# Tomsk-Smart-Tech/video-stream-segmenetation

Hardware: AMD Instinct MI355X
Metric: frames/sec (640×480, batch=8) at 1/2/4/8 MI355X + mask max-abs-err vs ref (higher is better)
Workload: dtype bf16; 1 GPU; 8 synthetic 640x480 RGB u8 frames per GPU per step (resident in HBM) -> 256x144 f32 masks, 4 steps in flight (one handle, 4 slots, 4 streams); global_batch=8, frame=640x480x3, model_res=256x144, pw_gemm=v_mfma_f32_16x16x32_bf16, f32 activations split hi+lo, graph=True, inflight=4, parallelism=dp1

## Files before the change

include/vss.h:

```cpp
#ifndef VSS_H_
#define VSS_H_

#include <stddef.h>
#include <stdint.h>

#ifdef __cplusplus
extern "C" {
#endif

#define VSS_VERSION 30000

enum {
  VSS_OK = 0,
  VSS_E_INVALID_ARG = -1,
  VSS_E_HIP = -2,
  VSS_E_RCCL = -3,
  VSS_E_BUSY = -4,
  VSS_E_OOM = -5,
  VSS_E_IO = -6,
  VSS_E_UNSUPPORTED = -7
};

enum {
  VSS_DTYPE_F32 = 0,
// ... 124 lines not shown
int vss_set_option(vss_handle* h, int option, int value);
int vss_get_option(vss_handle* h, int option, int* value);

int vss_layer_shape(const vss_handle* h, int layer, int* c, int* hh, int* ww);

int vss_read_layer(vss_handle* h, int layer, int n, float* host_out);

int vss_layer_kernel(const vss_handle* h, int layer, char* buf, int cap);

int vss_layer_tiles(const vss_handle* h, int layer, int* th, int* tw, int cap);

int vss_layer_tile_kernel(const vss_handle* h, int layer, int idx, char* buf, int cap);

int vss_layer_occupancy(const vss_handle* h, int layer, int* wg_per_cu, int* lds_bytes);

int vss_profile_read(vss_handle* h, double* ms_per_layer, int cap, int* count);

int vss_block_lds_bytes(int mode, int stride, int th, int tw, int cin, int cskip, int chid, int cout, int stem_in);

void vss_expand_frag_layout(int cin, int cout, int* out4);
int vss_expand_frag_image(int cin, int chid, int cout, int h0, int cs, const float* w1, const float* b1,
                          const float* wdw, const float* bdw, const float* w2, void* out);

typedef struct vss_post_config {
  double ema;
  double noise_cutoff;
  double high_threshold;
  double gamma;
  double sigma_spatial;
  double sigma_range;
  int use_bilateral;
} vss_post_config;

void vss_post_config_default(vss_post_config* cfg);

typedef struct vss_post_state vss_post_state;
int vss_post_create(vss_handle* h, const vss_post_config* cfg, vss_post_state** out);
void vss_post_destroy(vss_post_state* st);
int vss_post_reset(vss_post_state* st);
int vss_post_set_config(vss_post_state* st, const vss_post_config* cfg);

int vss_postprocess_device(vss_post_state* st, const uint8_t* d_frames, int n, int height, int width,
                           int channels, size_t row_stride, size_t frame_stride, const float* d_masks,
                           float* d_alpha, uint8_t* d_alpha_u8, void* stream);

typedef struct vss_face_frame {
// ... 54 lines not shown
```

video-stream-segmenetation_amd/__init__.py:

```python
from __future__ import annotations

import ctypes
import os
import subprocess
import threading
import weakref

import numpy as np

HERE = os.path.dirname(os.path.abspath(__file__))
LIB_PATH = os.environ.get("VSS_LIBRARY") or os.path.join(HERE, "lib", "libvss.so")
DEFAULT_WEIGHTS = os.path.join(HERE, "model", "vss_weights_seed7.bin")
HEADER = os.path.join(os.path.dirname(HERE), "include", "vss.h")

VSS_OK, VSS_E_INVALID_ARG, VSS_E_HIP, VSS_E_RCCL, VSS_E_BUSY, VSS_E_OOM, VSS_E_IO, VSS_E_UNSUPPORTED = (
    0, -1, -2, -3, -4, -5, -6, -7)
DTYPES = {"f32": 0, "bf16x2": 1}
VSS_OPT_USE_GRAPH, VSS_OPT_PROFILE, VSS_OPT_KEEP_STEM, VSS_OPT_ROW_FETCH = 1, 2, 6, 7
VSS_OPT_GRAPH_BUILDS, VSS_OPT_GRAPH_PATCHES, VSS_OPT_COMM_RANKS, VSS_OPT_GATHER_CALLS = 8, 9, 10, 11
VSS_OPT_GATHER_FORM = 12
VSS_GATHER_ORDERED, VSS_GATHER_CONCURRENT = 0, 1
GATHER_FORMS = {"ordered": VSS_GATHER_ORDERED, "concurrent": VSS_GATHER_CONCURRENT}
VSS_CREATE_NO_AUTOTUNE = 1
VSS_OUT_MODEL, VSS_OUT_FRAME = 0, 1
# ... 929 lines not shown


def shard_plan(n: int, nranks: int, rank: int):
    f, c, m = ctypes.c_int(), ctypes.c_int(), ctypes.c_int()
    _check(lib().vss_shard_plan(n, nranks, rank, ctypes.byref(f), ctypes.byref(c), ctypes.byref(m)))
    return f.value, c.value, m.value


def gather_runs(n: int, nranks: int):
    a, b, c = (ctypes.c_int * max(1, nranks))(), (ctypes.c_int * max(1, nranks))(), (ctypes.c_int * max(1, nranks))()
    k = lib().vss_gather_runs(n, nranks, a, b, c)
    _check(min(k, 0))
    return [(a[j], b[j], c[j]) for j in range(k)]


def version() -> int:
    return lib().vss_version()


def block_lds_bytes(mode, stride, th, tw, cin, cskip, chid, cout, stem_in=0) -> int:
    return lib().vss_block_lds_bytes(mode, stride, th, tw, cin, cskip, chid, cout, stem_in)


def expand_frag_layout(cin: int, cout: int) -> dict:
    out = (ctypes.c_int * 4)()
    lib().vss_expand_frag_layout(cin, cout, out)
    return dict(zip(("bytes", "aw", "f4s", "a2"), out))


def expand_frag_image(w1, b1, wdw, bdw, w2, h0: int = 0, cs: int | None = None) -> np.ndarray:
    arrs = [np.ascontiguousarray(a, np.float32) for a in (w1, b1, wdw, bdw, w2)]
    chid, cin = arrs[0].shape
    cout = arrs[4].shape[0]
    if arrs[1].shape != (chid,) or arrs[2].shape != (chid, 9) or arrs[3].shape != (chid,) or arrs[4].shape != (cout, chid):
        raise VssError(VSS_E_INVALID_ARG, "expand_frag_image: array shapes")
    cs = chid - h0 if cs is None else cs
    out = np.zeros((max(cs, 0) // 16, expand_frag_layout(cin, cout)["bytes"]), np.uint8)
    _check(lib().vss_expand_frag_image(cin, chid, cout, h0, cs, *[a.ctypes.data for a in arrs], out.ctypes.data))
    return out
```

video-stream-segmenetation_amd/csrc/vss_capi.hip:

```cpp
#include <hip/hip_ext.h>
#include <immintrin.h>

#include <chrono>
#include <cmath>
#include <cstdio>
#include <cstdlib>
#include <cstring>
#include <fstream>
#include <memory>

#include "vss_engine.h"

namespace vss {
void (*stem_kernel16())(StemParams);
void (*head_kernel16())(HeadParams);
void (*prep_kernel())(PrepParams);
}

using namespace vss;
using namespace vss_engine;

thread_local std::string vss_engine::g_tls_error;

namespace {
// ... 570 lines not shown
namespace {

StemParams stem_params(const vss_handle* h, const Slot& s, int li, const uint8_t* frames, size_t rs, size_t fs,
                       int fh, int fw, int fc) {
  const LayerPlan& l = h->L[li];
  const int Hm = h->cfg.model_h, Wm = h->cfg.model_w;
  StemParams p{};
  p.frames = frames; p.row_stride = (long)rs; p.frame_stride = (long)fs;
  p.fh = fh; p.fw = fw; p.fc = fc; p.Hm = Hm; p.Wm = Wm;
  p.ry = (float)((double)fh / (double)Hm);
  p.rx = (float)((double)fw / (double)Wm);
  p.w = l.stem_w; p.b = l.stem_b; p.y = s.act[li];
  p.Ho = l.H; p.Wo = l.W; p.cout = l.C;
  p.acc_zero = s.acc;
  p.acc_stride = h->acc_stride;
  return p;
}

BlockParams block_params(const vss_handle* h, const Slot& s, int li, int n, const LayerPlan* lp = nullptr) {
  const LayerPlan& l = lp ? *lp : h->L[li];
  const Rec& r = l.rec;
  const LayerPlan& src = h->L[r.src];
  BlockParams p{};
  p.wimg = l.wimg;
  p.wimg_stride = l.wimg_stride;
  p.wfrag = l.wfrag;
  p.wfrag_stride = l.wfrag_stride;
  p.x_part_stride = (long)src.part_stride;
  p.y_part_stride = (long)l.part_stride;
  p.x = s.act[r.src];
  p.y = s.act[li];
  p.eps = h->eps;
  p.N = n; p.H = l.inH; p.W = l.inW; p.Ho = l.H; p.Wo = l.W;
  p.cin = (int)r.cin; p.cout = l.C; p.chid = l.chid; p.stride = l.stride;
  p.TH = l.TH; p.TW = l.TW; p.tiles_x = l.tiles_x; p.tiles_y = l.tiles_y;
  p.acc_stride = h->acc_stride;
  if (r.kind == K_IR) {
    p.relu6_dw = 1;
    p.residual = (r.flags & F_RESIDUAL) ? 1 : 0;
  } else {
    const LayerPlan& sk = h->L[r.skip];
    p.skip = s.act[r.skip];
    p.skip_part_stride = (long)sk.part_stride;
    p.cskip = (int)r.chid;
    p.relu6_dw = 0;
    p.out_acc = s.acc + l.acc_off;
// ... 55 lines not shown
#endif
      L.fn = (const void*)lt.entry->fn[prec == PREC_F32 ? 0 : 1];
      L.grid = dim3(lt.tiles_x, lt.tiles_y, n * lt.ks);
      L.threads = lt.entry->threads;
      L.lds = lt.lds;
      L.prm.block = p;
    } else if (r.kind == K_HEAD) {
      const LayerPlan& src = h->L[r.src];
      HeadParams p{};
      p.x = s.act[r.src];
      p.in_acc = s.acc + src.acc_off;
      p.acc_stride = h->acc_stride;
      p.gamma = src.gamma; p.beta = src.beta; p.eps = h->eps;
      p.w = l.head_w; p.b = l.head_b; p.mask = masks;
      p.N = n; p.h = src.H; p.w_ = src.W; p.cin = src.C; p.Hm = Hm; p.Wm = Wm;
      p.inv_hw = 1.0 / ((double)src.H * src.W);
#ifdef VSS_TRACE
      p.trace = s.trace[i];
      h->trace_wgs[i] = ((Wm + kHeadTW - 1) / kHeadTW) * ((Hm + kHeadTH - 1) / kHeadTH) * n;
#endif
      L.fn = (const void*)head_kernel16();
      L.grid = dim3((Wm + kHeadTW - 1) / kHeadTW, (Hm + kHeadTH - 1) / kHeadTH, n);
      L.lds = kHeadLds * 4;
      L.prm.head = p;
    } else {
      continue;
    }
    out->push_back(L);
  }
}

hipKernelNodeParams node_params(const Launch& L, void** args) {
  hipKernelNodeParams kp{};
  args[0] = const_cast<Launch::Prm*>(&L.prm);
  kp.func = const_cast<void*>(L.fn);
  kp.gridDim = L.grid;
  kp.blockDim = dim3(L.threads);
  kp.sharedMemBytes = (unsigned)L.lds;
  kp.kernelParams = args;
  kp.extra = nullptr;
  return kp;
}

int launch_eager(vss_handle* h, const std::vector<Launch>& ls, hipStream_t st, int prof_slot) {
  const int nl = (int)h->L.size();
  for (const Launch& L : ls) {
// ... 11 lines not shown
  return VSS_OK;
}

int harvest_ring(vss_handle* h, int slot) {
  const int nl = (int)h->L.size();
  for (int i = 0; i < nl; ++i) {
    float ms = 0.f;
    if (h->L[i].fused) continue;
    HIP_TRY(h, hipEventSynchronize(h->ev[((size_t)slot * nl + i) * 2 + 1]));
    HIP_TRY(h, hipEventElapsedTime(&ms, h->ev[((size_t)slot * nl + i) * 2], h->ev[((size_t)slot * nl + i) * 2 + 1]));
    h->prof_sum[i] += ms;
  }
  h->prof_count++;
  h->ring_pending[slot] = 0;
  return VSS_OK;
}

bool has_fused_stem(const vss_handle* h) {
  for (const LayerPlan& l : h->L)
    if (flags_stem_in(l.flags)) return true;
  return false;
}

void destroy_graph(GraphEntry& g) {
  if (g.last && g.launched) (void)hipEventSynchronize(g.last);
  if (g.exec) (void)hipGraphExecDestroy(g.exec);
  if (g.graph) (void)hipGraphDestroy(g.graph);
  if (g.last) (void)hipEventDestroy(g.last);
  g = GraphEntry();
}

void destroy_graph_set(std::vector<GraphEntry>& v) {
  for (GraphEntry& g : v) destroy_graph(g);
  v.clear();
}

int build_graph(vss_handle* h, const std::vector<Launch>& ls, GraphEntry* out) {
  GraphEntry g;
  HIP_TRY(h, hipGraphCreate(&g.graph, 0));
  g.launches = ls;
  for (const Launch& L : g.launches) {
    void* args[1];
    const hipKernelNodeParams kp = node_params(L, args);
    hipGraphNode_t node = nullptr;
    const hipError_t e = hipGraphAddKernelNode(&node, g.graph, g.nodes.empty() ? nullptr : &g.nodes.back(),
                                               g.nodes.empty() ? 0 : 1, &kp);
    if (e != hipSuccess) {
      destroy_graph(g);
      return fail(h, VSS_E_HIP, std::string("hipGraphAddKernelNode: ") + hipGetErrorString(e));
    }
    g.nodes.push_back(node);
  }
  hipError_t e = hipGraphInstantiate(&g.exec, g.graph, nullptr, nullptr, 0);
  if (e == hipSuccess) e = hipEventCreateWithFlags(&g.last, hipEventDisableTiming);
  if (e != hipSuccess) {
    destroy_graph(g);
    return fail(h, VSS_E_HIP, std::string("hipGraphInstantiate: ") + hipGetErrorString(e));
  }
  h->graph_builds++;
  *out = std::move(g);
  return VSS_OK;
}

int graph_diff(const GraphEntry& g, const std::vector<Launch>& ls) {
  int d = 0;
  for (size_t i = 0; i < ls.size(); ++i) d += std::memcmp(&ls[i].prm, &g.launches[i].prm, sizeof(Launch::Prm)) != 0;
  return d;
}

int patch_graph(vss_handle* h, GraphEntry& g, const std::vector<Launch>& ls) {
  bool waited = false;
  for (size_t i = 0; i < ls.size(); ++i) {
    if (std::memcmp(&ls[i].prm, &g.launches[i].prm, sizeof(Launch::Prm)) == 0) continue;
    if (!waited && g.launched) HIP_TRY(h, hipEventSynchronize(g.last));
    waited = true;
    void* args[1];
    const hipKernelNodeParams kp = node_params(ls[i], args);
    HIP_TRY(h, hipGraphExecKernelNodeSetParams(g.exec, g.nodes[i], &kp));
    g.launches[i] = ls[i];
  }
  if (waited) h->graph_patches++;
  return VSS_OK;
}

constexpr size_t kMaxShapes = 16;
void make_room_for_shape(Slot& s) {
  if (s.graphs.size() < kMaxShapes) return;
  auto victim = s.graphs.begin();
  unsigned long long oldest = ~0ull;
  for (auto it = s.graphs.begin(); it != s.graphs.end(); ++it) {
    const auto t = s.shape_tick.find(it->first);
    const unsigned long long tick = t == s.shape_tick.end() ? 0ull : t->second;
    if (tick < oldest) {
      oldest = tick;
      victim = it;
    }
  }
  destroy_graph_set(victim->second);
  s.shape_tick.erase(victim->first);
  s.graphs.erase(victim);
}

int pick_graph(vss_handle* h, Slot& s, const GraphKey& key, const std::vector<Launch>& ls, GraphEntry** out) {
  auto it = s.graphs.find(key);
  if (it == s.graphs.end()) {
    make_room_for_shape(s);
    it = s.graphs.emplace(key, std::vector<GraphEntry>()).first;
  }
  s.shape_tick[key] = s.graph_tick + 1;
  std::vector<GraphEntry>& v = it->second;
  GraphEntry* lru = nullptr;
  for (GraphEntry& g : v) {
    if (graph_diff(g, ls) == 0) {
      *out = &g;
      return VSS_OK;
    }
    if (!lru || !g.launched || (lru->launched && g.tick < lru->tick)) lru = &g;
  }
  if ((int)v.size() < kExecPerShape && !(lru && !lru->launched)) {
    v.emplace_back();
    if (int rc = build_graph(h, ls, &v.back())) {
      v.pop_back();
      return rc;
    }
    *out = &v.back();
    return VSS_OK;
  }
  if (int rc = patch_graph(h, *lru, ls)) return rc;
  *out = lru;
  return VSS_OK;
}

struct DeviceClock {
  static constexpr int kPts = 8, kRing = 256;
  bool on = std::getenv("VSS_TIME_DEVICE") != nullptr;
  double t[kRing][kPts] = {};
  long calls = 0;
  double* cur = nullptr;
  static double now() {
    return std::chrono::duration<double, std::micro>(std::chrono::steady_clock::now().time_since_epoch()).count();
  }
  void begin() {
    if (!on) return;
    cur = t[calls++ % kRing];
    cur[0] = now();
  }
  void mark(int k) {
    if (on && cur) cur[k] = now();
  }
  void dump() {
    if (!on || !calls) return;
// ... 15 lines not shown
  h->last_n = n;
  h->last_slot = si;
  s.stem_stored = !has_fused_stem(h) || h->keep_stem;
  std::vector<Launch> ls;
  forward_launches(h, s, frames, n, fh, fw, fc, rs, fs, masks, &ls);
  g_device_clock.mark(3);
  if (h->profile) {
    const int ring = h->prof_next;
    h->prof_next = (h->prof_next + 1) % vss_handle::kProfRing;
    if (h->ring_pending[ring]) {
      int rc = harvest_ring(h, ring);
      if (rc) return rc;
    }
    int rc = launch_eager(h, ls, st, ring);
    if (!rc) h->ring_pending[ring] = 1;
    return rc;
  }
  if (!h->use_graph) return launch_eager(h, ls, st, -1);
  GraphEntry* g = nullptr;
  if (int rc = pick_graph(h, s, GraphKey{n, fh, fw, fc, rs, fs}, ls, &g)) return rc;
  g_device_clock.mark(4);
  HIP_TRY(h, hipGraphLaunch(g->exec, st));
  g_device_clock.mark(5);
  HIP_TRY(h, hipEventRecord(g->last, st));
  g_device_clock.mark(6);
  g->launched = true;
  g->tick = ++s.graph_tick;
  return VSS_OK;
}

void drop_graphs(vss_handle* h) {
  for (Slot& s : h->slots) {
    for (auto& kv : s.graphs) destroy_graph_set(kv.second);
    s.graphs.clear();
    s.shape_tick.clear();
  }
}

void enqueue_upmask(const vss_handle* h, const float* d_masks, int n, int fh, int fw, float* d_out, hipStream_t s) {
  UpmaskParams p{};
  p.masks = d_masks;
  p.H = h->cfg.model_h;
  p.W = h->cfg.model_w;
  p.sy = (float)p.H / (float)fh;
  p.sx = (float)p.W / (float)fw;
  p.out = d_out;
  p.fh = fh;
  p.fw = fw;
  launch_upmask(p, n, s);
}

std::vector<vss_handle*> engines(vss_handle* h) {
  std::vector<vss_handle*> e{h};
  e.insert(e.end(), h->peers.begin(), h->peers.end());
  return e;
}
// ... 588 lines not shown
    std::fprintf(stderr, "vss submit phases (us/call over %ld calls):", g_submit_clock.calls);
    for (int k = 0; k < SubmitClock::kPhases; ++k)
      std::fprintf(stderr, " %s %.1f", names[k], g_submit_clock.ns[k] / 1e3 / g_submit_clock.calls);
    std::fprintf(stderr, "\n");
    std::map<int, std::vector<std::vector<double>>> by_n;
    for (const auto& r : g_submit_clock.rows) by_n[r.first].push_back(r.second);
    for (auto& kv : by_n) {
      std::fprintf(stderr, "vss submit phases, %d-frame calls (%zu), median us:", kv.first, kv.second.size());
      for (int k = 0; k < SubmitClock::kPhases; ++k) {
        std::vector<double> v;
        for (const auto& r : kv.second) v.push_back(r[k]);
        std::nth_element(v.begin(), v.begin() + v.size() / 2, v.end());
        std::fprintf(stderr, " %s %.1f", names[k], v[v.size() / 2] / 1e3);
      }
      std::fprintf(stderr, "\n");
    }
    g_submit_clock = SubmitClock();
    g_submit_clock.on = true;
  }
  stop_completions(h);
  (void)hipSetDevice(h->device);
  (void)hipDeviceSynchronize();
  for (Slot& s : h->slots) {
    for (auto& kv : s.graphs) destroy_graph_set(kv.second);
    if (s.comm) (void)ncclCommDestroy(s.comm);
    if (s.stream) (void)hipStreamDestroy(s.stream);
    if (s.done) (void)hipEventDestroy(s.done);
    if (s.host_done) (void)hipEventDestroy(s.host_done);
  }
  for (auto e : h->ev)
    if (e) (void)hipEventDestroy(e);
  for (auto e : h->gather_ev)
    if (e) (void)hipEventDestroy(e);
  for (void* p : h->dev_allocs) (void)hipFree(p);
  for (void* p : h->host_allocs) (void)hipHostFree(p);
  if (h->stream) (void)hipStreamDestroy(h->stream);
  delete h->pool;
  delete h;
}

}

int vss_engine::segment_device_on(vss_handle* h, int* slot, const uint8_t* d_frames, int n, int height, int width,
                                  int channels, size_t row_stride, size_t frame_stride, float* d_masks,
                                  void* stream) {
  if (!h) return fail(nullptr, VSS_E_INVALID_ARG, "null handle");
  if (!d_frames || !d_masks) return fail(h, VSS_E_INVALID_ARG, "null device pointer");
// ... 508 lines not shown
      destroy_graph(g);
      return fail(h, VSS_E_HIP, std::string("hipGraphUpload: ") + hipGetErrorString(e));
    }
    HIP_TRY(h, hipStreamSynchronize(s.stream));
    s.graphs[key].push_back(std::move(g));
    s.shape_tick[key] = ++s.graph_tick;
  }
  return VSS_OK;
}

int vss_slot_stream(vss_handle* h, int k, void** stream) {
  if (!h || !stream) return fail(h, VSS_E_INVALID_ARG, "null handle/stream");
  if (k < 0 || k >= (int)h->slots.size()) return fail(h, VSS_E_INVALID_ARG, "slot out of range");
  *stream = h->slots[k].stream;
  return VSS_OK;
}

int vss_shard_plan(int n, int nranks, int rank, int* first, int* count, int* per_rank) {
  if (n < 0 || nranks < 1 || rank < 0 || rank >= nranks || !first || !count || !per_rank) return VSS_E_INVALID_ARG;
  shard_plan(n, nranks, rank, first, count, per_rank);
  return VSS_OK;
}

int vss_gather_runs(int n, int nranks, int* src_row, int* dst_row, int* rows) {
  if (n < 0 || nranks < 1 || !src_row || !dst_row || !rows) return VSS_E_INVALID_ARG;
  return gather_runs(n, nranks, src_row, dst_row, rows);
}

int vss_layer_shape(const vss_handle* h, int layer, int* c, int* hh, int* ww) {
  if (!h || layer < 0 || layer >= (int)h->L.size()) return VSS_E_INVALID_ARG;
  if (c) *c = h->L[layer].C;
  if (hh) *hh = h->L[layer].H;
  if (ww) *ww = h->L[layer].W;
  return VSS_OK;
}

int vss_layer_occupancy(const vss_handle* h, int layer, int* wg_per_cu, int* lds_bytes) {
  if (!h || layer < 0 || layer >= (int)h->L.size() || !wg_per_cu) return VSS_E_INVALID_ARG;
  const LayerPlan& l = h->L[layer];
  *wg_per_cu = 0;
  if (lds_bytes) *lds_bytes = (int)l.lds;
  if (!l.entry) return VSS_OK;
  const int pi = h->cfg.dtype == VSS_DTYPE_F32 ? 0 : 1;
  HIP_TRY(const_cast<vss_handle*>(h), hipSetDevice(h->device));
  HIP_TRY(const_cast<vss_handle*>(h),
          hipOccupancyMaxActiveBlocksPerMultiprocessor(wg_per_cu, (const void*)l.entry->fn[pi], l.entry->threads,
// ... 179 lines not shown
```

video-stream-segmenetation_amd/csrc/vss_engine.h:

```cpp
#pragma once

#include <hip/hip_runtime.h>
#include <rccl/rccl.h>

#include <algorithm>
#include <atomic>
#include <condition_variable>
#include <deque>
#include <functional>
#include <map>
#include <memory>
#include <mutex>
#include <string>
#include <thread>
#include <tuple>
#include <vector>

#include "../../include/vss.h"
#include "vss_kernels.h"

namespace vss_engine __attribute__((visibility("hidden"))) {

using namespace vss;

// ... 22 lines not shown
  const float *gamma = nullptr, *beta = nullptr;
  const float *stem_w = nullptr, *stem_b = nullptr, *head_w = nullptr;
  float head_b = 0.f;
};

struct Launch {
  const void* fn = nullptr;
  dim3 grid;
  int threads = kThreads;
  size_t lds = 0;
  int layer = 0;
  union Prm {
    StemParams stem;
    BlockParams block;
    HeadParams head;
  } prm;
};

using GraphKey = std::tuple<int, int, int, int, size_t, size_t>;
constexpr int kExecPerShape = 4;
struct GraphEntry {
  hipGraph_t graph = nullptr;
  hipGraphExec_t exec = nullptr;
  hipEvent_t last = nullptr;
  bool launched = false;
  unsigned long long tick = 0;
  std::vector<hipGraphNode_t> nodes;
  std::vector<Launch> launches;
};

struct RowPlan {
  std::vector<int> rows;
  std::vector<std::pair<int, int>> runs;
  int* d_rows = nullptr;
};

struct Slot {
  std::vector<float*> act;
  unsigned long long* acc = nullptr;
  float* d_masks = nullptr;
  float* d_gather = nullptr;
  hipStream_t stream = nullptr;
  hipEvent_t done = nullptr;
  hipStream_t done_stream = nullptr;
  hipEvent_t host_done = nullptr;
  bool used = false;
  bool leased = false;
// ... 343 lines not shown
```

video-stream-segmenetation_amd/csrc/vss_kernels.h:

```cpp
#pragma once
#include <cstddef>
#include <cstdint>

#include <hip/hip_runtime.h>

namespace vss {

enum Prec : int { PREC_F32 = 0, PREC_BF16X2 = 1, PREC_BF16 = 2 };

enum BlockMode : int { MODE_IR_EXPAND = 0, MODE_IR_DIRECT = 1, MODE_DEC = 2 };

__host__ __device__ constexpr int block_flags(int norm_in, int residual, int xp, int sp, int ks, int stem_in = 0) {
  return (norm_in ? 1 : 0) | (residual ? 2 : 0) | ((xp - 1) << 2) | ((sp - 1) << 4) | ((ks - 1) << 6) |
         (stem_in ? 256 : 0);
}
__host__ __device__ constexpr bool flags_stem_in(int f) { return (f & 256) != 0; }
__host__ __device__ constexpr int flags_xp(int f) { return ((f >> 2) & 3) + 1; }
__host__ __device__ constexpr int flags_sp(int f) { return ((f >> 4) & 3) + 1; }
__host__ __device__ constexpr int flags_ks(int f) { return ((f >> 6) & 3) + 1; }

constexpr int kThreads = 256;
constexpr int kLdsGranule = 2048, kLdsGranulesPerCu = 80;
__host__ __device__ constexpr int lds_wg_per_cu(int bytes) {
  return kLdsGranulesPerCu / ((bytes + kLdsGranule - 1) / kLdsGranule);
// ... 130 lines not shown
#define VSS_TRACE_FIELD unsigned long long* trace;
#define VSS_STAMP(k)                                                                                  \
  do {                                                                                                \
    if constexpr (!COH) {                                                                             \
      if (threadIdx.x == 0 && p.trace) {                                                              \
        unsigned long long* t_ = p.trace + (((long)blockIdx.z * gridDim.y + blockIdx.y) * gridDim.x + blockIdx.x) * 16; \
        t_[(k)] = __builtin_amdgcn_s_memrealtime();                                                   \
        t_[8 + (k)] = __builtin_amdgcn_s_memtime();                                                   \
        if ((k) == 0) {                                                                               \
                                    \
          t_[7] = __builtin_amdgcn_s_getreg((31 << 11) | 4);                                          \
          t_[15] = __builtin_amdgcn_s_getreg((15 << 11) | 20);                                        \
        }                                                                                             \
      }                                                                                               \
    }                                                                                                 \
  } while (0)
#else
#define VSS_TRACE_FIELD
#define VSS_STAMP(k) \
  do {               \
  } while (0)
#endif

struct StemParams {
  const uint8_t* frames;
  long row_stride, frame_stride;
  int fh, fw, fc;
  int Hm, Wm;
  float ry, rx;
  const float* w;
  const float* b;
  float* y;
  int Ho, Wo, cout;
  unsigned long long* acc_zero;
  int acc_stride;
  VSS_TRACE_FIELD
};

struct BlockParams {
  const float* wimg;
  long wimg_stride;
  const char* wfrag;
  long wfrag_stride;
  long x_part_stride;
  long skip_part_stride;
  long y_part_stride;
  const float* x;
  const float* skip;
  float* y;
  const unsigned long long* in_acc;
  const float* in_gamma;
  const float* in_beta;
  int in_hw;
  double in_inv_hw;
  unsigned long long* out_acc;
  int acc_stride;
  float eps;
  int N, H, W;
  int Ho, Wo;
  int cin, cskip, chid, cout;
  int stride;
  int relu6_dw;
// ... 24 lines not shown
  L.IW = TW + 2;
  L.P_IN = L.IH * L.IW;
  L.P_IN_PAD = (L.P_IN + 15) & ~15;
  L.XS = 16 + VSS_XS_PAD;
  L.XH = 2 * L.IH + 1;
  L.XW = 2 * L.IW + 1;
  L.XWP = L.XW + 1;
  int o = 0;
  L.x0 = o;  o += r4(3 * L.XH * L.XWP);
  L.sw = o;  o += 27 * 16;
  L.sb = o;  o += 16;
  L.xt = o;  o += r4(L.P_IN_PAD * L.XS);
  const BlockLds B = block_lds(1 , 1, TH, TW, 16, 0, 16, 16, 1);
  L.wim = o; o += B.wimg_end - B.w1;
  L.total = o;
  return L;
}
enum BlockVariant : int { VAR_BLOCK = 0, VAR_STEM_B1_WIDE = 1 };

const BlockEntry* block_registry(int* count);


struct HeadParams {
  const float* x;
  const unsigned long long* in_acc;
  int acc_stride;
  const float* gamma;
  const float* beta;
  float eps;
  double inv_hw;
  const float* w;
  float b;
  float* mask;
  int N, h, w_, cin;
  int Hm, Wm;
  VSS_TRACE_FIELD
};

constexpr int kStemTH = 8, kStemTW = 32, kStemIH = 2 * kStemTH + 1, kStemIWP = 2 * kStemTW + 2;
constexpr int kStemLds = r4(3 * kStemIH * kStemIWP) + 27 * 16 + 16;
constexpr int kHeadTH = 16, kHeadTW = 64, kHeadZR = 10, kHeadZC = 34, kHeadZCP = 35;
constexpr int kHeadLds = kAccSlots * 2 * 16 * 2 + r4(kHeadZR * kHeadZCP) + 3 * 16;

__host__ __device__ inline void norm_affine(unsigned long long s_fx, unsigned long long q_fx, double inv_hw,
                                            float eps, float gamma, float beta, float* scale, float* shift) {
  const double mean = (double)(long long)s_fx * (0x1p-32 * inv_hw);
// ... 312 lines not shown
};
void launch_nv12_unpack(const Nv12Params& p, int n, hipStream_t s);
void launch_nv12_pack(const Nv12Params& p, int n, hipStream_t s);

struct FetchRowsParams {
  const uint8_t* src;
  uint8_t* dst;
  const int* rows;
  long row_stride, frame_stride;
  int row_bytes;
  int vec16;
};
void launch_fetch_rows(const FetchRowsParams& p, int nrows, int nframes, hipStream_t s);

void launch_post_ema(const PostEmaParams& p, hipStream_t s);
void launch_post_filter(const PostFilterParams& p, int n, hipStream_t s);

#ifndef VSS_XCD_REMAP
#define VSS_XCD_REMAP 1
#endif
struct TileIdx {
  int x, y, z;
};
__device__ __forceinline__ TileIdx xcd_tile() {
  if constexpr (VSS_XCD_REMAP) {
    const int gx = (int)gridDim.x, gy = (int)gridDim.y;
    const int L = (int)blockIdx.x + gx * ((int)blockIdx.y + gy * (int)blockIdx.z);
    const int per = (gx * gy * (int)gridDim.z) >> 3;
    const int T = L < (per << 3) ? (L & 7) * per + (L >> 3) : L;
    const int zy = T / gx;
    return {T - zy * gx, zy % gy, zy / gy};
  } else {
    return {(int)blockIdx.x, (int)blockIdx.y, (int)blockIdx.z};
  }
}

}
```

video-stream-segmenetation_amd/csrc/vss_kernels.hip:

```cpp
#include <hip/hip_runtime.h>

#include <vector>

#include "vss_kernels.h"

namespace vss {

typedef float f4 __attribute__((ext_vector_type(4)));
typedef unsigned u4 __attribute__((ext_vector_type(4)));
typedef __bf16 bf4 __attribute__((ext_vector_type(4)));
typedef __bf16 bf8 __attribute__((ext_vector_type(8)));

__device__ __forceinline__ const void* uniform_ptr(const void* p) {
  const unsigned long long v = reinterpret_cast<unsigned long long>(p);
  const unsigned lo = __builtin_amdgcn_readfirstlane((unsigned)v);
  const unsigned hi = __builtin_amdgcn_readfirstlane((unsigned)(v >> 32));
  return reinterpret_cast<const void*>(((unsigned long long)hi << 32) | lo);
}

template <bool COH>
struct Gm {
  const float* b;
  __amdgpu_buffer_rsrc_t r;
  __device__ __forceinline__ explicit Gm(const float* base) : b(base) {
// ... 444 lines not shown
#define VSS_WDMA_FIRST 0
#endif
constexpr bool block_wdma(int mode, int wimg_f4) {
  return VSS_WDMA && (VSS_WDMA_ALL || mode == 2 || wimg_f4 >= 2560);
}
template <int N>
__device__ __forceinline__ void dma_f4(const f4* src, f4* dst) {
  const int lane = (int)threadIdx.x & 63;
  const int wb = __builtin_amdgcn_readfirstlane(((int)threadIdx.x >> 6) * 64);
  for (int o = wb; o < N; o += 256)
    if (N % 64 == 0 || o + lane < N)
      __builtin_amdgcn_global_load_lds((__attribute__((address_space(1))) void*)(src + o + lane),
                                       (__attribute__((address_space(3))) void*)(dst + o), 16, 0, 0);
}
struct NoStaged {
  template <class Load>
  __device__ __forceinline__ void issue(Load) {}
  template <class Store>
  __device__ __forceinline__ void commit(Store) const {}
};
template <bool ON>
__device__ __forceinline__ void dma_wait() {
  if constexpr (ON) asm volatile("s_waitcnt vmcnt(0)" ::: "memory");
}

template <bool B>
struct ChunkTag {
  static constexpr bool value = B;
};

template <int MODE, int STRIDE, int TH, int TW, int CIN, int CSKIP, int CH, int COUT, int FLAGS, int PREC, bool COH>
__device__ __forceinline__ void block_body(const BlockParams& p, int bx, int by, int bz, float* smem) {
  constexpr bool STEM_IN = flags_stem_in(FLAGS);
  constexpr BlockLds L = block_lds(MODE, STRIDE, TH, TW, CIN, CSKIP, CH, COUT, STEM_IN);
  constexpr bool NORM_IN = (FLAGS & 1) != 0, RES = (FLAGS & 2) != 0;
  constexpr int XP = flags_xp(FLAGS), SP = flags_sp(FLAGS), KS = flags_ks(FLAGS);
  static_assert(KS == 1 || MODE == MODE_IR_EXPAND, "only expand layers split their hidden channels");
  static_assert(SP == 1 || MODE == MODE_DEC, "skip parts: decoder only");
  constexpr int IW = L.IW, P_IN = L.P_in, P_IN_PAD = L.P_in_pad, P_OUT = L.P_out, XS = L.XS;
  constexpr int NCB = L.NCB, NPB = L.NPB, NCHUNK = L.NCHUNK, PW = L.PW, CS = L.CS, NPBW = L.NPBW;
  constexpr int RS = L.RS, SS = L.slab_stride;
  static_assert(L.NACC <= kMaxAcc, "too many accumulators per wave");
  static_assert(CIN % 16 == 0 && CH % 16 == 0 && COUT % 16 == 0 && P_OUT % 16 == 0, "shape");
  static_assert(MODE != MODE_IR_EXPAND || CIN <= 64, "expand cin <= 64");
  static_assert(!RES || (STRIDE == 1 && CIN == COUT && MODE != MODE_DEC), "residual shape");
  static_assert(MODE != MODE_IR_EXPAND || CS == 4, "expand deals its chunks to the 4 waves");
// ... 531 lines not shown
        }
#pragma unroll
        for (int j = 0; j < XR; ++j) {
          if constexpr (MODE == MODE_IR_DIRECT) a[j] = relu6v(a[j]);
          const f4 b = to_operand<PREC>(a[j]);
#pragma unroll
          for (int cb = 0; cb < NCB; ++cb) {
            f4& ac = acc[(q * XR + j) * NCB + cb];
            if constexpr (FIRST)
              ac = mma16_op<PREC>(f4{0.f, 0.f, 0.f, 0.f}, a2[cb], b);
            else
              ac = mma16_op<PREC>(ac, a2[cb], b);
          }
        }
      }
    };
    static_assert(CS <= NCHUNK, "every wave has a first chunk");
    dw_chunk(cw, ChunkTag<true>{});
    for (int ck = cw + CS; ck < NCHUNK; ck += CS) dw_chunk(ck, ChunkTag<false>{});
  }

  if constexpr (MODE == MODE_IR_DIRECT && CS == 1) {
    VSS_STAMP(2);
    const Gm<COH> gy(p.y + (long)n * Ho * Wo * COUT);
#pragma unroll
    for (int q = 0; q < NPBW / XR; ++q)
#pragma unroll
      for (int j = 0; j < XR; ++j) {
        const int pix = run_pix(pw + q * PW, j), ly = pix / TW, lx = pix % TW;
        const int oy = oy0 + ly, ox = ox0 + lx;
#pragma unroll
        for (int cb = 0; cb < NCB; ++cb) {
          f4 v = acc[(q * XR + j) * NCB + cb] + *reinterpret_cast<const f4*>(b2s + cb * 16 + 4 * g);
          if constexpr (RES) v = v + *reinterpret_cast<const f4*>(xt + xq((ly + 1) * IW + lx + 1, cb * 4 + g));
          if (oy < Ho && ox < Wo) gy.st(((long)oy * Wo + ox) * COUT + cb * 16 + 4 * g, v);
        }
      }
  } else {
  __syncthreads();
  VSS_STAMP(2);
  {
#pragma unroll
    for (int q = 0; q < NPBW / XR; ++q)
#pragma unroll
      for (int j = 0; j < XR; ++j)
#pragma unroll
        for (int cb = 0; cb < NCB; ++cb)
          *reinterpret_cast<f4*>(slabs + sq(cw, run_pix(pw + q * PW, j), cb * 4 + g)) = acc[(q * XR + j) * NCB + cb];
  }
  __syncthreads();
  constexpr int C4O = COUT / 4, NOUT = (P_OUT * C4O + 255) / 256;
  const Gm<COH> gy(p.y + ks * p.y_part_stride + (long)n * Ho * Wo * COUT);
  f4 outv[MODE == MODE_DEC ? NOUT : 1];
#pragma unroll
  for (int k = 0; k < NOUT; ++k) {
    const int i = tid + 256 * k;
    if (i < P_OUT * C4O) {
      const int pix = i / C4O, c4 = i % C4O;
      const int ly = pix / TW, lx = pix % TW;
      const int oy = oy0 + ly, ox = ox0 + lx;
      const bool valid = oy < Ho && ox < Wo;
      f4 v = *reinterpret_cast<const f4*>(slabs + sq(0, pix, c4));
#pragma unroll
      for (int s = 1; s < CS; ++s) v = v + *reinterpret_cast<const f4*>(slabs + sq(s, pix, c4));
      if (KS == 1 || ks == 0) {
        v = v + *reinterpret_cast<const f4*>(b2s + 4 * c4);
        if constexpr (RES) {
          if constexpr (MODE == MODE_IR_EXPAND)
            v = v + *reinterpret_cast<const f4*>(smem + L.xr + rq(pix, c4));
          else
            v = v + *reinterpret_cast<const f4*>(xt + xq((ly + 1) * IW + lx + 1, c4));
        }
      }
      if constexpr (MODE == MODE_DEC) {
        outv[k] = v;
// ... 62 lines not shown
    const Gm<COH> gst(p.stem.y + (long)n * p.H * p.W * 16);
    for (int i = tid; p.stem.y != nullptr && i < TH * TW * 4; i += 256) {
      const int pix = i >> 2, q = i & 3;
      const int yy = oy0 + pix / TW, xx = ox0 + pix % TW;
      if (yy < p.H && xx < p.W)
        gst.st(((long)yy * p.W + xx) * 16 + 4 * q,
               *reinterpret_cast<const f4*>(xt + xq((pix / TW + 1) * IW + pix % TW + 1, q)));
    }
  }
  VSS_STAMP(3);
}

constexpr int block_min_waves(int mode, int stride, int th, int tw, int cin, int cout, int prec) {
  if (mode != MODE_IR_EXPAND) return 1;
  const BlockLds L = block_lds(mode, stride, th, tw, cin, 0, 64, cout);
  if (tw != 8 || L.P_out > 32 || L.P_in_pad > 96 || L.NPB * L.NCB > 6) return 1;
  return prec == PREC_F32 ? (cin == 16 ? 4 : 3) : (cin == 16 ? 5 : 4);
}

template <int MODE, int STRIDE, int TH, int TW, int CIN, int CSKIP, int CH, int COUT, int FLAGS, int PREC>
__global__ __launch_bounds__(256) __attribute__((amdgpu_waves_per_eu(block_min_waves(MODE, STRIDE, TH, TW, CIN, COUT, PREC))))
void k_block(BlockParams p) {
  extern __shared__ __attribute__((aligned(16))) float smem[];
  const TileIdx t = xcd_tile();
  block_body<MODE, STRIDE, TH, TW, CIN, CSKIP, CH, COUT, FLAGS, PREC, false>(p, t.x, t.y, t.z, smem);
}

template <int TH, int TW, int PREC>
__global__ __launch_bounds__(kWideThreads) void k_stem_b1(BlockParams p) {
  extern __shared__ __attribute__((aligned(16))) float smem[];
  constexpr int WT = kWideThreads, NWAVE = WT / 64;
  constexpr StemB1Lds S = stem_b1_lds(TH, TW);
  constexpr int IH = S.IH, IW = S.IW, P_IN = S.P_IN, P_IN_PAD = S.P_IN_PAD, XS = S.XS;
  constexpr int XH = S.XH, XW = S.XW, XWP = S.XWP, NX = (XH * XW + WT - 1) / WT;
  constexpr BlockLds B = block_lds(MODE_IR_DIRECT, 1, TH, TW, 16, 0, 16, 16, 1);
  constexpr int WIMG4 = (B.wimg_end - B.w1) / 4;
  static_assert(WIMG4 <= WT && 27 * 16 <= WT, "one weight element per thread");
  float* x0s = smem + S.x0;
  float* sws = smem + S.sw;
  float* sbs = smem + S.sb;
  float* xt = smem + S.xt;
  float* wim = smem + S.wim;
  const TileIdx tl = xcd_tile();
  const int bx = tl.x, by = tl.y, n = tl.z;
  const int tid = threadIdx.x, lane = tid & 63, wave = tid >> 6, r = lane & 15, g = lane >> 4;
  const int oy0 = by * TH, ox0 = bx * TW, iy0 = oy0 - 1, ix0 = ox0 - 1;
  const StemParams& sp = p.stem;
  const int H = p.H, W = p.W;
  const uint8_t* fr = sp.frames + (long)n * sp.frame_stride;
  const int r0 = 2 * iy0 - 1, c0 = 2 * ix0 - 1;
  const f4 wv = reinterpret_cast<const f4*>(p.wimg)[min(tid, WIMG4 - 1)];
  const float swr = sp.w[min(tid, 27 * 16 - 1)];
  const float sb = sp.b[min(tid, 15)];
  uint32_t raw[NX][12];
  float dys[NX], dxs[NX];
#pragma unroll
  for (int u = 0; u < NX; ++u) {
    const int i = min(tid + WT * u, XH * XW - 1);
    const int ly = i / XW, lx = i - ly * XW;
    const int yy = min(max(r0 + ly, 0), sp.Hm - 1), xx = min(max(c0 + lx, 0), sp.Wm - 1);
    const PrepTap t = prep_tap(fr, sp.row_stride, sp.fc, sp.fh, sp.fw, sp.ry, sp.rx, yy, xx);
    prep_load(t, raw[u]);
    dys[u] = t.dy;
    dxs[u] = t.dx;
  }
  float o[NX][3];
// ... 150 lines not shown
#pragma unroll
    for (int dy = 0; dy < 2; ++dy) {
      float o[2];
#pragma unroll
      for (int dx = 0; dx < 2; ++dx) {
        const float v = dy == 0 ? __builtin_fmaf(0.75f, hz[1][dx], 0.25f * hz[0][dx])
                                : __builtin_fmaf(0.25f, hz[2][dx], 0.75f * hz[1][dx]);
        o[dx] = __builtin_amdgcn_rcpf(1.0f + __expf(-v));
      }
      if (oy + dy < p.Hm) {
        if (ox + 1 < p.Wm)
          *reinterpret_cast<float2*>(mrow + dy * p.Wm) = float2{o[0], o[1]};
        else if (ox < p.Wm)
          mrow[dy * p.Wm] = o[0];
      }
    }
  }
  VSS_STAMP(3);
}

template <int C>
__global__ __launch_bounds__(256) void k_head(HeadParams p) {
  extern __shared__ __attribute__((aligned(16))) float smem[];
  const TileIdx t = xcd_tile();
  head_body<C, false>(p, t.x, t.y, t.z, smem);
}

#ifndef VSS_SHARD
#define VSS_SHARD 0
#endif
#define VSS_BLOCK(M, S, TH, TW, CI, CK, CH, CO, FL)                                    \
  {M, S, TH, TW, CI, CK, CH, CO, FL,                                                  \
   {k_block<M, S, TH, TW, CI, CK, CH, CO, FL, PREC_F32>,                              \
    k_block<M, S, TH, TW, CI, CK, CH, CO, FL, PREC_BF16X2>}},
#define VSS_STR2(x) #x
#define VSS_STR(x) VSS_STR2(x)
#define VSS_CAT2(a, b) a##b
#define VSS_CAT(a, b) VSS_CAT2(a, b)
static const BlockEntry kShardBlocks[] = {
#include VSS_STR(VSS_CAT(vss_registry_, VSS_SHARD).inc)
};
#undef VSS_BLOCK

const BlockEntry* VSS_CAT(registry_shard_, VSS_SHARD)(int* count) {
  *count = (int)(sizeof(kShardBlocks) / sizeof(kShardBlocks[0]));
  return kShardBlocks;
}
// ... 36 lines not shown
```

Baseline: 245,900 frames/s.

## Precompute XCD tile map reciprocals, drop per-graph events, widen store coherence

Replaces the in-kernel integer divisions of the XCD tile remap with host-precomputed reciprocal multiply divmod passed in kernel params. It also removes the per-graph completion event, reusing the slot's done event for waits, which saves one event record per launch. It further changes output stores for small-COUT block layers to use the Gm store policy otherwise reserved for the COH flag, controlled by new macros. It adds Python/C APIs to inspect the tile map. The slot-level wait may block on more work than the single graph needed, and the changed store policy affects cache behaviour.

```diff
diff --git a/include/vss.h b/include/vss.h
--- a/include/vss.h
+++ b/include/vss.h
@@ -170,6 +170,9 @@
 int vss_expand_frag_image(int cin, int chid, int cout, int h0, int cs, const float* w1, const float* b1,
                           const float* wdw, const float* bdw, const float* w2, void* out);
 
+int vss_tile_map(int gx, int gy, int gz, unsigned* out6);
+int vss_tile_index(int gx, int gy, int gz, int* out);
+
 typedef struct vss_post_config {
   double ema;
   double noise_cutoff;
diff --git a/video-stream-segmenetation_amd/__init__.py b/video-stream-segmenetation_amd/__init__.py
--- a/video-stream-segmenetation_amd/__init__.py
+++ b/video-stream-segmenetation_amd/__init__.py
@@ -975,6 +975,22 @@
     return lib().vss_block_lds_bytes(mode, stride, th, tw, cin, cskip, chid, cout, stem_in)
 
 
+def tile_map(gx: int, gy: int, gz: int) -> dict:
+    out = (ctypes.c_uint * 6)()
+    fn = lib().vss_tile_map
+    fn.argtypes, fn.restype = [ctypes.c_int] * 3 + [ctypes.POINTER(ctypes.c_uint)], ctypes.c_int
+    _check(fn(gx, gy, gz, out))
+    return dict(zip(("gx", "gy", "rx", "ry", "per", "full"), out))
+
+
+def tile_index(gx: int, gy: int, gz: int) -> np.ndarray:
+    out = np.empty((3, gz * gy * gx), np.int32)
+    fn = lib().vss_tile_index
+    fn.argtypes, fn.restype = [ctypes.c_int] * 3 + [ctypes.c_void_p], ctypes.c_int
+    _check(fn(gx, gy, gz, out.ctypes.data))
+    return out
+
+
 def expand_frag_layout(cin: int, cout: int) -> dict:
     out = (ctypes.c_int * 4)()
     lib().vss_expand_frag_layout(cin, cout, out)
diff --git a/video-stream-segmenetation_amd/csrc/vss_capi.hip b/video-stream-segmenetation_amd/csrc/vss_capi.hip
--- a/video-stream-segmenetation_amd/csrc/vss_capi.hip
+++ b/video-stream-segmenetation_amd/csrc/vss_capi.hip
@@ -616,6 +616,7 @@
   const Rec& r = l.rec;
   const LayerPlan& src = h->L[r.src];
   BlockParams p{};
+  p.tm = tile_map((unsigned)l.tiles_x, (unsigned)l.tiles_y, (unsigned)(n * l.ks));
   p.wimg = l.wimg;
   p.wimg_stride = l.wimg_stride;
   p.wfrag = l.wfrag;
@@ -717,6 +718,7 @@
       L.fn = (const void*)head_kernel16();
       L.grid = dim3((Wm + kHeadTW - 1) / kHeadTW, (Hm + kHeadTH - 1) / kHeadTH, n);
       L.lds = kHeadLds * 4;
+      p.tm = tile_map(L.grid.x, L.grid.y, L.grid.z);
       L.prm.head = p;
     } else {
       continue;
@@ -774,16 +776,20 @@
   return false;
 }
 
-void destroy_graph(GraphEntry& g) {
-  if (g.last && g.launched) (void)hipEventSynchronize(g.last);
+int wait_slot_graphs(vss_handle* h, const Slot& s) {
+  if (s.used) HIP_TRY(h, hipEventSynchronize(s.done));
+  return VSS_OK;
+}
+
+void destroy_graph(GraphEntry& g, const Slot* s = nullptr) {
+  if (g.launched && s && s->used) (void)hipEventSynchronize(s->done);
   if (g.exec) (void)hipGraphExecDestroy(g.exec);
   if (g.graph) (void)hipGraphDestroy(g.graph);
-  if (g.last) (void)hipEventDestroy(g.last);
   g = GraphEntry();
 }
 
-void destroy_graph_set(std::vector<GraphEntry>& v) {
-  for (GraphEntry& g : v) destroy_graph(g);
+void destroy_graph_set(std::vector<GraphEntry>& v, const Slot& s) {
+  for (GraphEntry& g : v) destroy_graph(g, &s);
   v.clear();
 }
 
@@ -803,8 +809,7 @@
     }
     g.nodes.push_back(node);
   }
-  hipError_t e = hipGraphInstantiate(&g.exec, g.graph, nullptr, nullptr, 0);
-  if (e == hipSuccess) e = hipEventCreateWithFlags(&g.last, hipEventDisableTiming);
+  const hipError_t e = hipGraphInstantiate(&g.exec, g.graph, nullptr, nullptr, 0);
   if (e != hipSuccess) {
     destroy_graph(g);
     return fail(h, VSS_E_HIP, std::string("hipGraphInstantiate: ") + hipGetErrorString(e));
@@ -820,11 +825,12 @@
   return d;
 }
 
-int patch_graph(vss_handle* h, GraphEntry& g, const std::vector<Launch>& ls) {
+int patch_graph(vss_handle* h, const Slot& s, GraphEntry& g, const std::vector<Launch>& ls) {
   bool waited = false;
   for (size_t i = 0; i < ls.size(); ++i) {
     if (std::memcmp(&ls[i].prm, &g.launches[i].prm, sizeof(Launch::Prm)) == 0) continue;
-    if (!waited && g.launched) HIP_TRY(h, hipEventSynchronize(g.last));
+    if (!waited && g.launched)
+      if (int rc = wait_slot_graphs(h, s)) return rc;
     waited = true;
     void* args[1];
     const hipKernelNodeParams kp = node_params(ls[i], args);
@@ -848,7 +854,7 @@
       victim = it;
     }
   }
-  destroy_graph_set(victim->second);
+  destroy_graph_set(victim->second, s);
   s.shape_tick.erase(victim->first);
   s.graphs.erase(victim);
 }
@@ -878,7 +884,7 @@
     *out = &v.back();
     return VSS_OK;
   }
-  if (int rc = patch_graph(h, *lru, ls)) return rc;
+  if (int rc = patch_graph(h, s, *lru, ls)) return rc;
   *out = lru;
   return VSS_OK;
 }
@@ -940,7 +946,6 @@
   g_device_clock.mark(4);
   HIP_TRY(h, hipGraphLaunch(g->exec, st));
   g_device_clock.mark(5);
-  HIP_TRY(h, hipEventRecord(g->last, st));
   g_device_clock.mark(6);
   g->launched = true;
   g->tick = ++s.graph_tick;
@@ -949,7 +954,7 @@
 
 void drop_graphs(vss_handle* h) {
   for (Slot& s : h->slots) {
-    for (auto& kv : s.graphs) destroy_graph_set(kv.second);
+    for (auto& kv : s.graphs) destroy_graph_set(kv.second, s);
     s.graphs.clear();
     s.shape_tick.clear();
   }
@@ -1584,7 +1589,7 @@
   (void)hipSetDevice(h->device);
   (void)hipDeviceSynchronize();
   for (Slot& s : h->slots) {
-    for (auto& kv : s.graphs) destroy_graph_set(kv.second);
+    for (auto& kv : s.graphs) destroy_graph_set(kv.second, s);
     if (s.comm) (void)ncclCommDestroy(s.comm);
     if (s.stream) (void)hipStreamDestroy(s.stream);
     if (s.done) (void)hipEventDestroy(s.done);
@@ -2139,6 +2144,29 @@
   return VSS_OK;
 }
 
+int vss_tile_map(int gx, int gy, int gz, unsigned* out6) {
+  if (gx < 1 || gy < 1 || gz < 1 || !out6 || (long long)gx * gy * gz > 0x7FFFFFFFll) return VSS_E_INVALID_ARG;
+  const TileMap m = tile_map((unsigned)gx, (unsigned)gy, (unsigned)gz);
+  const unsigned v[6] = {m.gx, m.gy, m.rx, m.ry, m.per, m.full};
+  std::memcpy(out6, v, sizeof v);
+  return VSS_OK;
+}
+
+int vss_tile_index(int gx, int gy, int gz, int* out) {
+  if (gx < 1 || gy < 1 || gz < 1 || !out || (long long)gx * gy * gz > 0x7FFFFFFFll) return VSS_E_INVALID_ARG;
+  const TileMap m = tile_map((unsigned)gx, (unsigned)gy, (unsigned)gz);
+  const size_t n = (size_t)gx * gy * gz;
+  for (int bz = 0; bz < gz; ++bz)
+    for (int by = 0; by < gy; ++by)
+      for (int bx = 0; bx < gx; ++bx, ++out) {
+        const TileIdx t = tile_of(m, (unsigned)bx, (unsigned)by, (unsigned)bz);
+        out[0] = t.x;
+        out[n] = t.y;
+        out[2 * n] = t.z;
+      }
+  return VSS_OK;
+}
+
 int vss_gather_runs(int n, int nranks, int* src_row, int* dst_row, int* rows) {
   if (n < 0 || nranks < 1 || !src_row || !dst_row || !rows) return VSS_E_INVALID_ARG;
   return gather_runs(n, nranks, src_row, dst_row, rows);
diff --git a/video-stream-segmenetation_amd/csrc/vss_engine.h b/video-stream-segmenetation_amd/csrc/vss_engine.h
--- a/video-stream-segmenetation_amd/csrc/vss_engine.h
+++ b/video-stream-segmenetation_amd/csrc/vss_engine.h
@@ -68,7 +68,6 @@
 struct GraphEntry {
   hipGraph_t graph = nullptr;
   hipGraphExec_t exec = nullptr;
-  hipEvent_t last = nullptr;
   bool launched = false;
   unsigned long long tick = 0;
   std::vector<hipGraphNode_t> nodes;
diff --git a/video-stream-segmenetation_amd/csrc/vss_kernels.h b/video-stream-segmenetation_amd/csrc/vss_kernels.h
--- a/video-stream-segmenetation_amd/csrc/vss_kernels.h
+++ b/video-stream-segmenetation_amd/csrc/vss_kernels.h
@@ -176,6 +176,13 @@
   } while (0)
 #endif
 
+struct TileMap {
+  unsigned gx, gy;
+  unsigned rx, ry;
+  unsigned per;
+  unsigned full;
+};
+
 struct StemParams {
   const uint8_t* frames;
   long row_stride, frame_stride;
@@ -192,6 +199,7 @@
 };
 
 struct BlockParams {
+  TileMap tm;
   const float* wimg;
   long wimg_stride;
   const char* wfrag;
@@ -262,6 +270,7 @@
 
 
 struct HeadParams {
+  TileMap tm;
   const float* x;
   const unsigned long long* in_acc;
   int acc_stride;
@@ -620,17 +629,34 @@
 struct TileIdx {
   int x, y, z;
 };
-__device__ __forceinline__ TileIdx xcd_tile() {
+__host__ __device__ inline unsigned tile_recip(unsigned d) {
+  const unsigned long long m = 0x100000000ull / d;
+  return m > 0xFFFFFFFFull ? 0xFFFFFFFFu : (unsigned)m;
+}
+__host__ __device__ inline TileMap tile_map(unsigned gx, unsigned gy, unsigned gz) {
+  const unsigned per = (gx * gy * gz) >> 3;
+  return {gx, gy, tile_recip(gx), tile_recip(gy), per, per << 3};
+}
+__host__ __device__ __forceinline__ void tile_divmod(unsigned T, unsigned d, unsigned m, unsigned& q, unsigned& r) {
+  q = (unsigned)(((unsigned long long)T * m) >> 32);
+  r = T - q * d;
+  if (r >= d) {
+    ++q;
+    r -= d;
+  }
+}
+__host__ __device__ __forceinline__ TileIdx tile_of(const TileMap& m, unsigned bx, unsigned by, unsigned bz) {
   if constexpr (VSS_XCD_REMAP) {
-    const int gx = (int)gridDim.x, gy = (int)gridDim.y;
-    const int L = (int)blockIdx.x + gx * ((int)blockIdx.y + gy * (int)blockIdx.z);
-    const int per = (gx * gy * (int)gridDim.z) >> 3;
-    const int T = L < (per << 3) ? (L & 7) * per + (L >> 3) : L;
-    const int zy = T / gx;
-    return {T - zy * gx, zy % gy, zy / gy};
+    const unsigned L = bx + m.gx * (by + m.gy * bz);
+    const unsigned T = L < m.full ? (L & 7) * m.per + (L >> 3) : L;
+    unsigned zy, x, z, y;
+    tile_divmod(T, m.gx, m.rx, zy, x);
+    tile_divmod(zy, m.gy, m.ry, z, y);
+    return {(int)x, (int)y, (int)z};
   } else {
-    return {(int)blockIdx.x, (int)blockIdx.y, (int)blockIdx.z};
+    return {(int)bx, (int)by, (int)bz};
   }
 }
-
-}
+__device__ __forceinline__ TileIdx xcd_tile(const TileMap& m) { return tile_of(m, blockIdx.x, blockIdx.y, blockIdx.z); }
+
+}
diff --git a/video-stream-segmenetation_amd/csrc/vss_kernels.hip b/video-stream-segmenetation_amd/csrc/vss_kernels.hip
--- a/video-stream-segmenetation_amd/csrc/vss_kernels.hip
+++ b/video-stream-segmenetation_amd/csrc/vss_kernels.hip
@@ -490,6 +490,20 @@
 template <bool ON>
 __device__ __forceinline__ void dma_wait() {
   if constexpr (ON) asm volatile("s_waitcnt vmcnt(0)" ::: "memory");
+}
+
+#ifndef VSS_WT_COUT_MAX
+#define VSS_WT_COUT_MAX 32
+#endif
+#ifndef VSS_WT_MODES
+#define VSS_WT_MODES 7
+#endif
+#ifndef VSS_WT_RES
+#define VSS_WT_RES 0
+#endif
+constexpr bool block_wt_stores(int mode, int stride, int cout) {
+  return cout <= VSS_WT_COUT_MAX && ((VSS_WT_MODES >> mode) & 1) &&
+         (VSS_WT_RES || !(mode == MODE_IR_EXPAND && stride == 1));
 }
 
 template <bool B>
@@ -1067,7 +1081,7 @@
 
   if constexpr (MODE == MODE_IR_DIRECT && CS == 1) {
     VSS_STAMP(2);
-    const Gm<COH> gy(p.y + (long)n * Ho * Wo * COUT);
+    const Gm<COH || block_wt_stores(MODE, STRIDE, COUT)> gy(p.y + (long)n * Ho * Wo * COUT);
 #pragma unroll
     for (int q = 0; q < NPBW / XR; ++q)
 #pragma unroll
@@ -1095,7 +1109,7 @@
   }
   __syncthreads();
   constexpr int C4O = COUT / 4, NOUT = (P_OUT * C4O + 255) / 256;
-  const Gm<COH> gy(p.y + ks * p.y_part_stride + (long)n * Ho * Wo * COUT);
+  const Gm<COH || block_wt_stores(MODE, STRIDE, COUT)> gy(p.y + ks * p.y_part_stride + (long)n * Ho * Wo * COUT);
   f4 outv[MODE == MODE_DEC ? NOUT : 1];
 #pragma unroll
   for (int k = 0; k < NOUT; ++k) {
@@ -1204,7 +1218,7 @@
 __global__ __launch_bounds__(256) __attribute__((amdgpu_waves_per_eu(block_min_waves(MODE, STRIDE, TH, TW, CIN, COUT, PREC))))
 void k_block(BlockParams p) {
   extern __shared__ __attribute__((aligned(16))) float smem[];
-  const TileIdx t = xcd_tile();
+  const TileIdx t = xcd_tile(p.tm);
   block_body<MODE, STRIDE, TH, TW, CIN, CSKIP, CH, COUT, FLAGS, PREC, false>(p, t.x, t.y, t.z, smem);
 }
 
@@ -1223,7 +1237,7 @@
   float* sbs = smem + S.sb;
   float* xt = smem + S.xt;
   float* wim = smem + S.wim;
-  const TileIdx tl = xcd_tile();
+  const TileIdx tl = xcd_tile(p.tm);
   const int bx = tl.x, by = tl.y, n = tl.z;
   const int tid = threadIdx.x, lane = tid & 63, wave = tid >> 6, r = lane & 15, g = lane >> 4;
   const int oy0 = by * TH, ox0 = bx * TW, iy0 = oy0 - 1, ix0 = ox0 - 1;
@@ -1420,7 +1434,7 @@
 template <int C>
 __global__ __launch_bounds__(256) void k_head(HeadParams p) {
   extern __shared__ __attribute__((aligned(16))) float smem[];
-  const TileIdx t = xcd_tile();
+  const TileIdx t = xcd_tile(p.tm);
   head_body<C, false>(p, t.x, t.y, t.z, smem);
 }
 
```

After: 265,800 frames/s (median of 6 runs). 8.1% higher.
